# Zhengjun-Du/LC-CRF-SLAM

Hardware: AMD Instinct MI355X
Metric: CRF mean-field iters/sec (higher is better)
Workload: dtype f32; 1 GPU; C2: 2000 keypoints, 5 iters, two 2-D kernels (TUM3.yaml), L=2; frames_in_flight_per_gpu=16384, handles=1, distinct_frames=64, n_points=2000, n_iters=5, n_labels=2, engine=fused

## Files before the change

lc-crf-slam_amd/csrc/fused_lean.h:

```cpp
#pragma once

#include "fused_loop.h"

#ifndef LCCRF_LEAN_SKIP
#define LCCRF_LEAN_SKIP 0
#endif
#define LEAN_SKIP(bit) ((LCCRF_LEAN_SKIP & (bit)) != 0)

namespace lccrf {
namespace fl {

constexpr int kLeanMaxRounds = 4;
__host__ __device__ constexpr int lean_rounds(int nt) { return nt >= 512 ? 3 : 4; }
__host__ __device__ constexpr int lean_max_v(int nt) { return 3 * (nt - 64); }

__host__ __device__ inline int lean_plane_floats(int NA, int V0)
{
    const int top = V0 < kChainTop ? V0 : kChainTop;
    return (NA * kD1 + 11 * top + 3 * (V0 - top) + 16 + 63) & ~63;
}

__host__ __device__ inline bool lean_chain_wanted(int NA, int V0, int row0, int nt)
{
    return row0 >= kChainMinRow && V0 <= chain_max_v(nt) && V0 <= 256 && lean_plane_floats(NA, V0) < 65535;
}

struct LeanTables {
    int val0, val1, nbr, row;
};
__host__ __device__ inline LeanTables lean_tables(size_t &o, int Vk, bool chain)
{
    auto take = [&](size_t bytes) { size_t r = o; o += (bytes + 15) & ~(size_t)15; return (int)r; };
    LeanTables t;
    t.val0 = take((size_t)(Vk + 1) * sizeof(float2));
    t.val1 = take((size_t)(Vk + 1) * sizeof(float2));
    t.nbr = chain ? take((size_t)kD1 * Vk * sizeof(unsigned)) : -1;
    t.row = take((size_t)(Vk + 2) * sizeof(unsigned short));
    return t;
}

__host__ __device__ inline bool layout_lean(int NA, int K, const int *V, int row0, FusedLayout *lay, int nt, size_t lds_limit)
{
    constexpr int D1 = kD1;
    if (NA < 1 || K < 1 || K > kMaxFusedK) return false;
    for (int k = 0; k < K; ++k)
        if (V[k] >= 65535 || V[k] > lean_max_v(nt)) return false;
    if (row0 >= kChainMinRow && !lean_chain_wanted(NA, V[0], row0, nt)) return false;
    const int chain0 = lean_chain_wanted(NA, V[0], row0, nt);
    {
        FusedLayout L{};
        size_t o = 0;
        auto take = [&](size_t bytes) { size_t r = o; o += (bytes + 15) & ~(size_t)15; return (int)r; };
        L.prod_all = 0;
        L.chain0 = chain0;
        L.zero = take(128);
        size_t shared_prod = 0;
        for (int k = 0; k < K; ++k) {
            const bool chain = k == 0 && chain0;
            L.Ecap[k] = chain ? lean_plane_floats(NA, V[k]) : ((NA * D1 + 63) & ~63);
            const LeanTables lt = lean_tables(o, V[k], chain);
            L.val[k][0] = lt.val0;
            L.val[k][1] = lt.val1;
            L.nbr[k] = lt.nbr;
            L.row[k] = lt.row;
            const size_t pb = (size_t)L.Ecap[k] * 2 * sizeof(float);
            shared_prod = pb > shared_prod ? pb : shared_prod;
        }
        if (o > 65535) return false;
        L.pstart = chain0 ? take((size_t)(V[0] + 2) * sizeof(unsigned short)) : 0;
        const int p = take(shared_prod < 1024 ? 1024 : shared_prod);
        for (int k = 0; k < K; ++k) L.prod[k] = p;
        L.total = (int)o;
        if (o <= lds_limit) {
            *lay = L;
            return true;
        }
    }
    return false;
}

#define LCCRF_ASM_SEL(off, vlo, vhi, S)                                                                             \
    "v_cmp_lt_i32_e32 vcc, " #off ", %[rem]\n\tv_cndmask_b32_e32 %[" #S "], 0, %[ad], vcc\n\t"                     \
    "ds_read_b128 v[" #vlo ":" #vhi "], %[" #S "] offset:" #off "\n\t"

__device__ __forceinline__ float chain_rows_sel(unsigned addr, int bytes, unsigned trips, unsigned &keep0, unsigned &keep1)
{
    float acc = 0.0f;
    if (trips == 0) return acc;
    unsigned sa, sb;
    asm volatile(
        LCCRF_ASM_SEL(0, 96, 99, sa) LCCRF_ASM_SEL(16, 100, 103, sb)
        LCCRF_ASM_SEL(32, 104, 107, sa) LCCRF_ASM_SEL(48, 108, 111, sb)
        LCCRF_ASM_SEL(64, 112, 115, sa) LCCRF_ASM_SEL(80, 116, 119, sb)
        "1:\n\t"
        LCCRF_ASM_SEL(96, 120, 123, sa) LCCRF_ASM_SEL(112, 124, 127, sb)
        "s_waitcnt lgkmcnt(6)\n\t"
        LCCRF_ASM_ADD8(v96, v97, v98, v99, v100, v101, v102, v103)
        "v_add_u32_e32 %[ad], 0x80, %[ad]\n\t"
        "v_subrev_u32_e32 %[rem], 0x80, %[rem]\n\t"
        LCCRF_ASM_SEL(0, 96, 99, sa) LCCRF_ASM_SEL(16, 100, 103, sb)
        "s_waitcnt lgkmcnt(6)\n\t"
        LCCRF_ASM_ADD8(v104, v105, v106, v107, v108, v109, v110, v111)
        LCCRF_ASM_SEL(32, 104, 107, sa) LCCRF_ASM_SEL(48, 108, 111, sb)
        "s_waitcnt lgkmcnt(6)\n\t"
        LCCRF_ASM_ADD8(v112, v113, v114, v115, v116, v117, v118, v119)
        LCCRF_ASM_SEL(64, 112, 115, sa) LCCRF_ASM_SEL(80, 116, 119, sb)
        "s_waitcnt lgkmcnt(6)\n\t"
        LCCRF_ASM_ADD8(v120, v121, v122, v123, v124, v125, v126, v127)
        "s_sub_u32 %[n], %[n], 1\n\t"
        "s_cmp_lg_u32 %[n], 0\n\t"
        "s_cbranch_scc1 1b\n\t"
        "s_waitcnt lgkmcnt(0)\n\t"
        : [acc] "+v"(acc), [ad] "+v"(addr), [rem] "+v"(bytes), [n] "+s"(trips), [sa] "=&v"(sa), [sb] "=&v"(sb), "+v"(keep0), "+v"(keep1)
        :
        : "scc", "vcc", "memory", LCCRF_CHAIN_RING_CLOBBERS);
    return acc;
}

__device__ __forceinline__ float chain_rows_keep(unsigned addr, unsigned end, unsigned trips, unsigned &keep0, unsigned &keep1)
{
    float acc = 0.0f;
    if (trips == 0) return acc;
    const unsigned e1 = end - 32u, e2 = end - 64u, e3 = end - 96u;
    unsigned sel;
    asm volatile(LCCRF_CHAIN_ROWS_ASM
                 : [acc] "+v"(acc), [ad] "+v"(addr), [n] "+s"(trips), [sel] "=&v"(sel), "+v"(keep0), "+v"(keep1)
                 : [e0] "v"(end), [e1] "v"(e1), [e2] "v"(e2), [e3] "v"(e3)
                 : "scc", "memory", LCCRF_CHAIN_RING_CLOBBERS);
    return acc;
}

__device__ __forceinline__ float2 lds_f2(unsigned addr)
{
#if defined(__HIP_DEVICE_COMPILE__)
    typedef float lean_f2 __attribute__((ext_vector_type(2)));
    const lean_f2 v = *reinterpret_cast<const __attribute__((address_space(3))) lean_f2 *>((unsigned long)addr);
    return make_float2(v.x, v.y);
#else
    (void)addr;
    return make_float2(0.f, 0.f);
#endif
}

__device__ __forceinline__ void lds_store_f(unsigned addr, float v)
{
#if defined(__HIP_DEVICE_COMPILE__)
    *reinterpret_cast<__attribute__((address_space(3))) float *>((unsigned long)addr) = v;
#else
    (void)addr; (void)v;
#endif
}
__device__ __forceinline__ void lds_store_f2(unsigned addr, float a, float b)
{
#if defined(__HIP_DEVICE_COMPILE__)
    typedef float lean_f2 __attribute__((ext_vector_type(2)));
    lean_f2 v;
    v.x = a;
    v.y = b;
    *reinterpret_cast<__attribute__((address_space(3))) lean_f2 *>((unsigned long)addr) = v;
#else
    (void)addr; (void)a; (void)b;
#endif
}

template <int PPT, int K, int CH>
__device__ __forceinline__ void point_products_lean(const FusedLayout &lay, const PointRegs<PPT, K> &pr, int s, int k)
{
    const unsigned a0 = (pr.ix[s][k][1] >> 16) << 2, a1 = (pr.ix[s][k][2] & 0xffffu) << 2, a2 = (pr.ix[s][k][2] >> 16) << 2;
    if (chain_k<CH>(lay, k)) {
        const unsigned pb = (unsigned)lay.Ecap[k] * 4u;
        lds_store_f(a0, pr.bary[s][k][0] * pr.q[s].x);
        lds_store_f(a0 + pb, pr.bary[s][k][0] * pr.q[s].y);
        lds_store_f(a1, pr.bary[s][k][1] * pr.q[s].x);
        lds_store_f(a1 + pb, pr.bary[s][k][1] * pr.q[s].y);
        lds_store_f(a2, pr.bary[s][k][2] * pr.q[s].x);
        lds_store_f(a2 + pb, pr.bary[s][k][2] * pr.q[s].y);
    } else {
        lds_store_f2(a0, pr.bary[s][k][0] * pr.q[s].x, pr.bary[s][k][0] * pr.q[s].y);
        lds_store_f2(a1, pr.bary[s][k][1] * pr.q[s].x, pr.bary[s][k][1] * pr.q[s].y);
        lds_store_f2(a2, pr.bary[s][k][2] * pr.q[s].x, pr.bary[s][k][2] * pr.q[s].y);
    }
}

template <int PPT, int K>
__device__ __forceinline__ float2 slice_point_lean(const PointRegs<PPT, K> &pr, int s, int k, float alpha)
{
    const float2 x0 = lds_f2(pr.ix[s][k][0] & 0xffffu), x1 = lds_f2(pr.ix[s][k][0] >> 16), x2 = lds_f2(pr.ix[s][k][1] & 0xffffu);
    const float w0 = pr.bary[s][k][0] * alpha, w1 = pr.bary[s][k][1] * alpha, w2 = pr.bary[s][k][2] * alpha;
    float t0 = w0 * x0.x, t1 = w0 * x0.y;
    t0 += w1 * x1.x; t1 += w1 * x1.y;
    t0 += w2 * x2.x; t1 += w2 * x2.y;
    return make_float2(t0, t1);
}

template <int NT>
__device__ __forceinline__ ChainLane chain_setup_lean(unsigned char *smem, const FusedLayout &lay, int V0, int tid)
{
    constexpr int k = 0;
    ChainLane cl{0u, 0u};
    int *hist = reinterpret_cast<int *>(smem + lay.prod[k]);
    if (tid < 128) hist[tid] = 0;
    __syncthreads();
    const unsigned short *row = reinterpret_cast<const unsigned short *>(smem + lay.row[k]);
    unsigned short *srt = reinterpret_cast<unsigned short *>(smem + lay.prod[k]) + 256;
    unsigned short *pstart = reinterpret_cast<unsigned short *>(smem + lay.pstart);
    int key = 0;
    if (tid < V0) {
        const int len = (int)row[tid + 1] - (int)row[tid];
        key = 63 - min((len + 3) >> 4, 63);
        atomicAdd(&hist[key], 1);
    }
    __syncthreads();
    if (tid < 64) {
        const int x = hist[tid];
        int incl = x;
#pragma unroll
        for (int o = 1; o < 64; o <<= 1) {
            const int y = __shfl_up(incl, o, 64);
            if (tid >= o) incl += y;
        }
        hist[64 + tid] = incl - x;
    }
    __syncthreads();
    if (tid < V0) srt[atomicAdd(&hist[64 + key], 1)] = (unsigned short)tid;
    __syncthreads();
    if (tid < 64) {
        int sz[4], sum = 0;
#pragma unroll
        for (int u = 0; u < 4; ++u) {
            const int r = tid * 4 + u;
            sz[u] = 0;
            if (r < V0) {
                const int v = srt[r];
                const int rl = (int)row[v + 1] - (int)row[v];
                sz[u] = ((rl + 3) & ~3) + (r < kChainTop ? 8 : 0);
            }
            sum += sz[u];
        }
        int incl = sum;
#pragma unroll
        for (int o = 1; o < 64; o <<= 1) {
            const int y = __shfl_up(incl, o, 64);
            if (tid >= o) incl += y;
        }
        int base = incl - sum;
#pragma unroll
        for (int u = 0; u < 4; ++u) {
            const int r = tid * 4 + u;
            if (r < V0) pstart[srt[r]] = (unsigned short)base;
            base += sz[u];
        }
    }
    __syncthreads();
    const int l = (tid >> 6) & 1, pr = tid >> 7, ln = tid & 63;
    const int r = pr == 0 ? (chain_top_rank(ln) >= 0 ? chain_top_rank(ln) : V0) : kChainTop + ((pr - 1) << 6) + ln;
    unsigned quads = 0, addr = 0;
    if (r < V0) {
        const int v = srt[r];
        const int rl = (int)row[v + 1] - (int)row[v], len4 = (rl + 3) & ~3;
        addr = (unsigned)(lay.prod[k] + 4 * (l * lay.Ecap[k] + (int)pstart[v]));
        quads = (unsigned)(len4 >> 2);
        cl.b = quads | ((unsigned)(len4 - rl) << 13) | ((unsigned)((v + 1) * 2 + l) << 16);
    }
    unsigned m = quads;
#pragma unroll
    for (int o = 32; o > 0; o >>= 1) m = max(m, (unsigned)__shfl_xor((int)m, o));
    cl.a = addr | (m << 18);
    __syncthreads();
    return cl;
}

__device__ __forceinline__ void chain_pads_lean(unsigned char *smem, const ChainLane &cl, int tid)
{
    if (cl.b >> 16) {
        float *e = reinterpret_cast<float *>(smem + (cl.a & 0x3ffffu)) + (cl.b & 0x1fffu) * 4u;
        const unsigned npad = (cl.b >> 13) & 3u;
        for (unsigned z = 1; z <= npad; ++z) e[-(int)z] = 0.0f;
        if ((tid >> 7) == 0) {
            reinterpret_cast<float4 *>(e)[0] = make_float4(0.f, 0.f, 0.f, 0.f);
            reinterpret_cast<float4 *>(e)[1] = make_float4(0.f, 0.f, 0.f, 0.f);
        }
    }
}

template <int PPT, int K, int CH, int NT>
__device__ __forceinline__ void place_products_lean(unsigned char *smem, const FusedLayout &lay, int N, int tid,
                                                    const unsigned (&pk)[PPT][K][kD1], PointRegs<PPT, K> &pr)
{
#pragma unroll
    for (int k = 0; k < K; ++k) {
        const unsigned short *row = reinterpret_cast<const unsigned short *>(smem + lay.row[k]);
        const unsigned short *pstart = reinterpret_cast<const unsigned short *>(smem + lay.pstart);
#pragma unroll
        for (int s = 0; s < PPT; ++s) {
            const unsigned vb = (unsigned)lay.val[k][kD1 & 1];
            pr.ix[s][k][0] = (vb + 8u * (pk[s][k][0] & 0xffffu)) | ((vb + 8u * (pk[s][k][1] & 0xffffu)) << 16);
            pr.ix[s][k][1] = vb + 8u * (pk[s][k][2] & 0xffffu);
            pr.ix[s][k][2] = 0;
            if (tid + s * NT < N) {
                unsigned sl[kD1];
#pragma unroll
                for (int j = 0; j < kD1; ++j) {
                    sl[j] = pk[s][k][j] >> 16;
                    if (chain_k<CH>(lay, k)) {
                        const int v = (int)(pk[s][k][j] & 0xffffu) - 1;
                        sl[j] = (unsigned)((int)pstart[v] + ((int)(pk[s][k][j] >> 16) - (int)row[v]));
                        sl[j] = ((unsigned)lay.prod[k] >> 2) + sl[j];
                    } else {
                        sl[j] = ((unsigned)lay.prod[k] >> 2) + 2u * sl[j];
                    }
                }
                pr.ix[s][k][1] |= sl[0] << 16;
                pr.ix[s][k][2] = sl[1] | (sl[2] << 16);
            }
        }
    }
}

__host__ __device__ inline int lean_sorted_vertex(int q, int V, int nt)
{
    const int r = q / nt;
    int w = (q % nt) >> 6;
    if ((r & 1) && (r + 1) * nt <= V) w = (nt >> 6) - 1 - w;
    return r * nt + (w << 6) + (q & 63);
}

template <int NT>
__device__ __forceinline__ int block_excl_scan(int x, int tid, int *ws)
{
    int incl = x;
#pragma unroll
    for (int o = 1; o < 64; o <<= 1) {
        const int y = __shfl_up(incl, o, 64);
        if ((tid & 63) >= o) incl += y;
    }
    if ((tid & 63) == 63) ws[tid >> 6] = incl;
    __syncthreads();
    int before = 0;
#pragma unroll
    for (int w = 0; w < NT / 64; ++w) {
        const int s = ws[w];
        if (w < (tid >> 6)) before += s;
    }
    return before + incl - x;
}

template <int PPT, int K, int NT>
__device__ __forceinline__ void sort_short_rows(unsigned char *smem, const FusedLayout &lay, int k, int Vk, int tid,
                                                unsigned (&pk)[PPT][K][kD1], const unsigned *gnbr, int Epad, unsigned *out, int axis_words)
{
    constexpr int VM = (lean_max_v(NT) + 8 + 7) & ~7;
    static_assert(NT == 512, "one lane per (bucket, segment): 64 x 8");
    static_assert(4 * VM * 2 + 64 <= ((NT * kD1 + 63) & ~63) * 8, "the scratch fits the smallest product buffer of the plan");
    unsigned short *row = reinterpret_cast<unsigned short *>(smem + lay.row[k]);
    unsigned short *key = reinterpret_cast<unsigned short *>(smem + lay.prod[k]);
    unsigned short *perm = key + VM, *nlen = perm + VM, *nrow = nlen + VM;
    int *ws = reinterpret_cast<int *>(nrow + VM);
    __syncthreads();
    for (int v = tid; v < Vk; v += NT) key[v] = (unsigned short)(63 - min((int)row[v + 1] - (int)row[v], 63));
    __syncthreads();
    const int b = tid >> 3, seg_len = (Vk + 7) >> 3, lo = min((tid & 7) * seg_len, Vk), hi = min(lo + seg_len, Vk);
    int cnt = 0;
    for (int v = lo; v < hi; ++v) cnt += key[v] == b ? 1 : 0;
    int q = block_excl_scan<NT>(cnt, tid, ws);
    for (int v = lo; v < hi; ++v) {
        if (key[v] == b) {
            const int nv = lean_sorted_vertex(q++, Vk, NT);
            perm[v] = (unsigned short)nv;
            nlen[nv] = (unsigned short)((int)row[v + 1] - (int)row[v]);
        }
    }
    __syncthreads();
    {
        int l[3], sum = 0;
#pragma unroll
        for (int i = 0; i < 3; ++i) {
            l[i] = tid * 3 + i < Vk ? (int)nlen[tid * 3 + i] : 0;
            sum += l[i];
        }
        int at = block_excl_scan<NT>(sum, tid, ws + NT / 64);
#pragma unroll
        for (int i = 0; i < 3; ++i) {
            if (tid * 3 + i <= Vk) nrow[tid * 3 + i] = (unsigned short)at;
            at += l[i];
        }
    }
    __syncthreads();
#pragma unroll
    for (int s = 0; s < PPT; ++s) {
#pragma unroll
        for (int j = 0; j < kD1; ++j) {
            const unsigned w = pk[s][k][j], id = w & 0xffffu;
            if (id) {
                const int v = (int)id - 1, nv = perm[v];
                pk[s][k][j] = (unsigned)(nv + 1) | ((unsigned)((int)nrow[nv] + ((int)(w >> 16) - (int)row[v])) << 16);
            }
        }
    }
    for (int j = 0; j < kD1; ++j) {
        for (int v = tid; v < Vk; v += NT) {
            const unsigned n = gnbr[(size_t)j * Epad + v], n1 = n & 0xffffu, n2 = n >> 16;
            out[j * axis_words + perm[v]] = (n1 ? (unsigned)perm[n1 - 1] + 1u : 0u) | ((n2 ? (unsigned)perm[n2 - 1] + 1u : 0u) << 16);
        }
    }
    __syncthreads();
    for (int v = tid; v <= Vk; v += NT) row[v] = nrow[v];
    __syncthreads();
}

typedef unsigned lean_u3 __attribute__((ext_vector_type(3)));
struct LeanSrc {
    __amdgpu_buffer_rsrc_t nbr[kMaxFusedK];
    __amdgpu_buffer_rsrc_t bary[kMaxFusedK];
    __amdgpu_buffer_rsrc_t norm[kMaxFusedK];
    __amdgpu_buffer_rsrc_t unary;
    int nbr_axis_bytes[kMaxFusedK];
    int off_nbr[kMaxFusedK], off_bary[kMaxFusedK], off_norm[kMaxFusedK], off_unary;
};
constexpr int kLeanRecPoints = 4 * kNTSmall;
constexpr int kLeanRecUnary = 0;
constexpr int kLeanRecBary = kLeanRecUnary + kLeanRecPoints * 8;
constexpr int kLeanRecNorm = kLeanRecBary + kMaxFusedK * kLeanRecPoints * kD1 * 4;
constexpr int kLeanRecNbr = kLeanRecNorm + kMaxFusedK * kLeanRecPoints * 4;
constexpr int kLeanRecNbrAxis = lean_max_v(kNTSmall) * 4;
constexpr int kLeanRecBytes = (kLeanRecNbr + kD1 * kLeanRecNbrAxis + 255) & ~255;
__device__ __forceinline__ __amdgpu_buffer_rsrc_t lean_rsrc(const void *p, size_t bytes)
{
    return __builtin_amdgcn_make_buffer_rsrc(const_cast<void *>(p), 0, (int)bytes, 0x00020000);
}

template <int PPT, int K>
__device__ __forceinline__ void opaque_ids(PointRegs<PPT, K> &pr)
{
#pragma unroll
    for (int s = 0; s < PPT; ++s) {
#pragma unroll
        for (int k = 0; k < K; ++k) asm volatile("" : "+v"(pr.ix[s][k][0]), "+v"(pr.ix[s][k][1]), "+v"(pr.ix[s][k][2]));
    }
}

struct LeanPrepPlan {
    int cl_off;
    int row_off[kMaxFusedK], row_bytes[kMaxFusedK];
    int nbr_off[kMaxFusedK], nbr_bytes[kMaxFusedK];
    int snbr_off[kMaxFusedK], snbr_axis[kMaxFusedK];
    int total;
};
constexpr unsigned kLeanPrepFormat = 7;
__host__ __device__ inline LeanPrepPlan lean_prep_plan(const FusedLayout &lay, int K, const int *Vcap, int nt, int ppt, bool sorted = false)
{
    LeanPrepPlan p{};
    int o = K * ppt * nt * 12;
    p.cl_off = o;
    o += nt * 8;
    for (int k = 0; k < K; ++k) {
        p.row_off[k] = o;
        p.row_bytes[k] = ((Vcap[k] + 2) * 2 + 15) & ~15;
        o += p.row_bytes[k];
        p.nbr_off[k] = o;
        p.nbr_bytes[k] = lay.nbr[k] >= 0 ? ((kD1 * Vcap[k] * 4 + 15) & ~15) : 0;
        o += p.nbr_bytes[k];
    }
    for (int k = 0; k < K; ++k) {
        p.snbr_off[k] = o;
        p.snbr_axis[k] = (sorted && lay.nbr[k] < 0) ? ((Vcap[k] + 3) & ~3) * 4 : 0;
        o += kD1 * p.snbr_axis[k];
    }
    p.total = (o + 255) & ~255;
    return p;
}

template <int PPT, int K, int CH, int NT, bool RELOAD, bool NORM = false, bool PRELOADED = false>
__device__ __forceinline__ void mean_field_lean(unsigned char *smem, const FusedLayout &lay, const int (&V)[K], int N, int &t,
                                                PointRegs<PPT, K> &pr, ChainLane &cl, const float (&alpha)[K],
                                                const float (&wk)[K], const LeanSrc &src, int n_iter, float relax, float omr, Instr &ins)
{
    constexpr int D1 = kD1;
    constexpr int KF = K - 1;
    const int wave_base = __builtin_amdgcn_readfirstlane(t & ~63);
    (void)wave_base;
#define LEAN_FRESH_T()                                                                                               \
    do {                                                                                                             \
        int z_ = 0;                                                                                                  \
        asm volatile("" : "+v"(z_));                                                                                 \
        t = wave_base + (int)__builtin_amdgcn_mbcnt_hi(~0u, __builtin_amdgcn_mbcnt_lo(~0u, (unsigned)z_));          \
    } while (0)
    auto load_weights = [&]() {
        if (!RELOAD) return;
#pragma unroll
        for (int s = 0; s < PPT; ++s) {
            const int i = t + s * NT;
            if (!NORM) {
                typedef unsigned lean_u2 __attribute__((ext_vector_type(2)));
                const lean_u2 u = __builtin_amdgcn_raw_buffer_load_b64(src.unary, i * 8, src.off_unary, 0);
                pr.un[s] = make_float2(__uint_as_float(u.x), __uint_as_float(u.y));
            }
#pragma unroll
            for (int k = 0; k < K; ++k) {
                const lean_u3 b = __builtin_amdgcn_raw_buffer_load_b96(src.bary[k], i * (D1 * 4), src.off_bary[k], 0);
                pr.bary[s][k][0] = __uint_as_float(b.x);
                pr.bary[s][k][1] = __uint_as_float(b.y);
                pr.bary[s][k][2] = __uint_as_float(b.z);
                if (!NORM) pr.wn[s][k] = __uint_as_float(__builtin_amdgcn_raw_buffer_load_b32(src.norm[k], i * 4, src.off_norm[k], 0));
            }
        }
        if (NORM) return;
#pragma unroll
        for (int s = 0; s < PPT; ++s)
#pragma unroll
            for (int k = 0; k < K; ++k) pr.wn[s][k] = wk[k] * pr.wn[s][k];
    };
    auto phase_P = [&](int k) {
#pragma unroll
        for (int s = 0; s < PPT; ++s)
            if (t + s * NT < N) point_products_lean<PPT, K, CH>(lay, pr, s, k);
        if (chain_k<CH>(lay, k)) chain_pads_lean(smem, cl, t);
    };
    auto phase_S = [&](int k) {
        float *val = reinterpret_cast<float *>(smem + lay.val[k][0]);
        if (chain_k<CH>(lay, k)) {
            const int npairs = 1 + ((max(V[k] - kChainTop, 0) + 63) >> 6);
            if (__builtin_expect((t >> 7) < npairs, 1)) {
                FL_PSTAMP();
                if ((t >> 7) == 0) __builtin_amdgcn_s_setprio(3);
                asm volatile("" : "+v"(cl.a), "+v"(cl.b));
                if (__builtin_expect((cl.b >> 16) != 0, 1) && !LEAN_SKIP(2)) {
                    const unsigned row_addr = cl.a & 0x3ffffu, row_end = row_addr + (cl.b & 0x1fffu) * 16u;
                    const unsigned m = (unsigned)__builtin_amdgcn_readfirstlane((int)(cl.a >> 18));
                    const float acc = (t >> 7) == 0 ? chain_rows_keep(row_addr, row_end, (((m + 1u) >> 1) + 3u) >> 2, cl.a, cl.b)
                                                      : chain_rows_sel(row_addr, (int)((cl.b & 0x1fffu) * 16u), (m + 7u) >> 3, cl.a, cl.b);
                    val[cl.b >> 16] = acc;
                }
                LEAN_FRESH_T();
                if ((t >> 7) == 0) __builtin_amdgcn_s_setprio(0);
                FL_PSTAMP();
            }
            return;
        }
        if (LEAN_SKIP(32)) return;
        const float2 *pl = reinterpret_cast<const float2 *>(smem + lay.prod[k]);
        const float2 *zero = reinterpret_cast<const float2 *>(smem + lay.zero);
        const unsigned short *row = reinterpret_cast<const unsigned short *>(smem + lay.row[k]);
        constexpr int RS = (K == 2 && CH == 0) ? 1 : lean_rounds(NT);
        for (int base = 0; base < lean_rounds(NT); base += RS) {
            int p0[RS], pe[RS];
#pragma unroll
            for (int r = 0; r < RS; ++r) {
                const int v = t + (base + r) * NT;
                p0[r] = pe[r] = 0;
                if (v < V[k]) { p0[r] = row[v]; pe[r] = row[v + 1]; }
            }
            float2 x[RS][8];
#pragma unroll
            for (int r = 0; r < RS; ++r) {
                const unsigned base = (unsigned)lay.prod[k] + 8u * (unsigned)p0[r];
                const int n = pe[r] - p0[r];
#pragma unroll
                for (int u = 0; u < 8; ++u) x[r][u] = lds_f2(((u < n) ? base : 0u) + 8u * u);
            }
#pragma unroll
            for (int r = 0; r < RS; ++r) {
                const int v = t + (base + r) * NT;
                float a0 = 0.0f, a1 = 0.0f;
#pragma unroll
                for (int u = 0; u < 8; ++u) { a0 += x[r][u].x; a1 += x[r][u].y; }
                for (int p = p0[r] + 8; p < pe[r] && !LEAN_SKIP(16); p += 8) {
                    float2 y[8];
#pragma unroll
                    for (int u = 0; u < 8; ++u) y[u] = *((p + u < pe[r]) ? pl + p + u : zero);
#pragma unroll
                    for (int u = 0; u < 8; ++u) { a0 += y[u].x; a1 += y[u].y; }
                }
                if (v < V[k]) reinterpret_cast<float2 *>(val)[v + 1] = make_float2(a0, a1);
            }
        }
        (void)V;
    };
    constexpr int R = lean_rounds(NT);
    constexpr int OVL_K = (K == 2 && CH == 1) ? 1 : K;
    auto load_nbr = [&](unsigned (&w)[OVL_K][D1][R]) {
#pragma unroll
        for (int k = 0; k < K; ++k) {
#pragma unroll
            for (int j = 0; j < D1; ++j) {
#pragma unroll
                for (int r = 0; r < R; ++r) {
                    w[k][j][r] = 0;
                    if (!(CH == 1 && k == 0) && (r == 0 || r * NT < V[k]))
                        w[k][j][r] = __builtin_amdgcn_raw_buffer_load_b32(src.nbr[k], (t + r * NT) * 4, src.off_nbr[k] + j * src.nbr_axis_bytes[k], 0);
                }
            }
        }
    };
    auto blur_pass = [&](int j, const unsigned (&w)[OVL_K][D1][R]) {
#pragma unroll
        for (int k = 0; k < K; ++k) {
            const float2 *src_v = reinterpret_cast<const float2 *>(smem + lay.val[k][j & 1]);
            float2 *dst = reinterpret_cast<float2 *>(smem + lay.val[k][(j & 1) ^ 1]);
            const bool in_lds = CH == 1 && k == 0;
            const unsigned *lds = reinterpret_cast<const unsigned *>(smem + (in_lds ? lay.nbr[k] : 0)) + j * V[k];
#pragma unroll
            for (int r = 0; r < (in_lds ? 1 : R); ++r) {
                const int v = t + r * NT;
                if (v < V[k]) {
                    const unsigned n = in_lds ? lds[v] : w[k][j][r];
                    const float2 o = src_v[v + 1], x = src_v[n & 0xffffu], y = src_v[n >> 16];
                    float2 u;
                    u.x = o.x + 0.5f * (x.x + y.x);
                    u.y = o.y + 0.5f * (x.y + y.y);
                    dst[v + 1] = u;
                }
            }
        }
    };
    constexpr bool OVL = K == 2 && CH == 1;
    constexpr int NA0 = NT - 128, RA = 4;
    constexpr int NB = NT - 64, RB = 3;
    auto load_nbr_ovl = [&](unsigned (&wa)[RA], unsigned (&wb)[2][RB]) {
#pragma unroll
        for (int r = 0; r < RA; ++r) {
            wa[r] = 0;
            if ((r == 0 || r * NA0 < V[K - 1]) && !LEAN_SKIP(512))
                wa[r] = __builtin_amdgcn_raw_buffer_load_b32(src.nbr[K - 1], (t - 128 + r * NA0) * 4, src.off_nbr[K - 1], 0);
        }
#pragma unroll
        for (int j = 1; j < D1; ++j) {
#pragma unroll
            for (int r = 0; r < RB; ++r) {
                wb[j - 1][r] = 0;
                if ((r == 0 || r * NB < V[K - 1]) && !LEAN_SKIP(512))
                    wb[j - 1][r] = __builtin_amdgcn_raw_buffer_load_b32(src.nbr[K - 1], (t + r * NB) * 4, src.off_nbr[K - 1] + j * src.nbr_axis_bytes[K - 1], 0);
            }
        }
    };
    auto blur_vertex = [&](const float2 *src_v, float2 *dst, int v, unsigned n) {
        if (LEAN_SKIP(64)) return;
        const float2 o = src_v[v + 1], x = src_v[n & 0xffffu], y = src_v[n >> 16];
        float2 u;
        u.x = o.x + 0.5f * (x.x + y.x);
        u.y = o.y + 0.5f * (x.y + y.y);
        dst[v + 1] = u;
    };
    auto blur_big = [&](int j, int lane, int stride, int rounds, const unsigned *w) {
        constexpr int k = K - 1;
        const float2 *src_v = reinterpret_cast<const float2 *>(smem + lay.val[k][j & 1]);
        float2 *dst = reinterpret_cast<float2 *>(smem + lay.val[k][(j & 1) ^ 1]);
#pragma unroll
        for (int r = 0; r < RA; ++r) {
            if (r < rounds) {
                const int v = lane + r * stride;
                if (v < V[k]) blur_vertex(src_v, dst, v, w[r]);
            }
        }
    };
    auto blur_small = [&](int lane, int j_lo, int j_hi) {
        const unsigned *tbl = reinterpret_cast<const unsigned *>(smem + lay.nbr[0]);
#pragma unroll
        for (int j = 0; j < D1; ++j) {
            if (j < j_lo || j >= j_hi) continue;
            const float2 *src_v = reinterpret_cast<const float2 *>(smem + lay.val[0][j & 1]);
            float2 *dst = reinterpret_cast<float2 *>(smem + lay.val[0][(j & 1) ^ 1]);
            for (int v = lane; v < V[0]; v += 64) blur_vertex(src_v, dst, v, tbl[j * V[0] + v]);
            asm volatile("s_waitcnt lgkmcnt(0)" ::: "memory");
            __builtin_amdgcn_wave_barrier();
        }
    };
    auto point_update = [&](int s) {
        if constexpr (NORM) {
#pragma unroll
            for (int k = 0; k < K; ++k) {
                const float v = slice_point_lean(pr, s, k, alpha[k]).x;
                const float nrm = 1.0f / (v + 1e-20f);
                if (RELOAD) __builtin_amdgcn_raw_buffer_store_b32(__float_as_uint(nrm), src.norm[k], (t + s * NT) * 4, src.off_norm[k], 0);
                else pr.wn[s][k] = wk[k] * nrm;
            }
            return;
        }
        float nx[2] = {-pr.un[s].x, -pr.un[s].y};
#pragma unroll
        for (int k = 0; k < K; ++k) {
            const float2 t = slice_point_lean(pr, s, k, alpha[k]);
            nx[0] += pr.wn[s][k] * t.x;
            nx[1] += pr.wn[s][k] * t.y;
        }
        pr.q[s] = softmax2(nx[0], nx[1], pr.q[s], relax, omr);
    };

    if (n_iter <= 0) return;
    if (!PRELOADED) load_weights();
#pragma unroll
    for (int s = 0; s < PPT; ++s)
        if (t + s * NT < N) point_products_lean<PPT, K, CH>(lay, pr, s, KF);
    if (chain_k<CH>(lay, KF)) chain_pads_lean(smem, cl, t);
    for (int it = 0; it < n_iter; ++it) {
        LEAN_FRESH_T();
        if (RELOAD) opaque_ids(pr);
        else opaque(pr);
        unsigned w[OVL ? 1 : K][D1][R];
        unsigned wa[RA], wb[2][RB];
        if constexpr (OVL) load_nbr_ovl(wa, wb);
        else load_nbr(w);
        __syncthreads();
        FL_STAMP();
        phase_S(KF);
#pragma unroll
        for (int k = KF - 1; k >= 0; --k) {
            __syncthreads();
            opaque_ids(pr);
            phase_P(k);
            __syncthreads();
            phase_S(k);
        }
        if constexpr (OVL) {
            if (t >= 128) blur_big(0, t - 128, NA0, RA, wa);
            __syncthreads();
            FL_STAMP();
            LEAN_FRESH_T();
            if (t >= NB) blur_small(t - NB, 0, 2);
            else blur_big(1, t, NB, RB, wb[0]);
            __syncthreads();
            if (!NORM && !LEAN_SKIP(256)) load_weights();
            if (t < NB) blur_big(2, t, NB, RB, wb[1]);
            else blur_small(t - NB, 2, D1);
            __syncthreads();
        } else {
            __syncthreads();
            FL_STAMP();
            LEAN_FRESH_T();
            blur_pass(0, w);
            __syncthreads();
            blur_pass(1, w);
            __syncthreads();
            if (!NORM && !LEAN_SKIP(256)) load_weights();
            blur_pass(2, w);
            __syncthreads();
        }
        FL_STAMP();
        LEAN_FRESH_T();
        opaque_ids(pr);
        const bool more = it + 1 < n_iter;
#pragma unroll
        for (int s = 0; s < PPT; ++s) {
            if (t + s * NT < N && !LEAN_SKIP(128)) {
                point_update(s);
                if (more) point_products_lean<PPT, K, CH>(lay, pr, s, KF);
            }
        }
        FL_STAMP();
    }
}

#undef LEAN_FRESH_T

}
}
```

Baseline: 49.93 million iters/s.

## Split chain rows across one wave with half-wave lanes, freeing a wave for blur

Remaps the chain-sum (phase_S) work so that each 64-lane wave handles 32 chain rows, two lanes per row for the two labels, instead of a wave pair covering 64 rows. The chain therefore uses one wave for the top rows rather than two. The first blur pass on the other lattice can then start at thread 64 instead of 128 and needs three rounds instead of four. This is meant to put more threads on the overlapped blur and shorten the critical path. In exchange each chain lane handles fewer distinct rows, and the prep format version is bumped because the lane layout changed.

Result: faster. 50.57 million iters/s, median of 6 (+1.3%).

```diff
diff --git a/lc-crf-slam_amd/csrc/fused_lean.h b/lc-crf-slam_amd/csrc/fused_lean.h
--- a/lc-crf-slam_amd/csrc/fused_lean.h
+++ b/lc-crf-slam_amd/csrc/fused_lean.h
@@ -10,13 +10,18 @@
 namespace lccrf {
 namespace fl {
 
+#ifndef LCCRF_CHAIN_TOP
+#define LCCRF_CHAIN_TOP 16
+#endif
+constexpr int kLeanChainTop = LCCRF_CHAIN_TOP;
+static_assert(kLeanChainTop == kChainTop || kLeanChainTop == 32, "16 rows on the lanes chain_top_rank names, or a full wavefront");
 constexpr int kLeanMaxRounds = 4;
 __host__ __device__ constexpr int lean_rounds(int nt) { return nt >= 512 ? 3 : 4; }
 __host__ __device__ constexpr int lean_max_v(int nt) { return 3 * (nt - 64); }
 
 __host__ __device__ inline int lean_plane_floats(int NA, int V0)
 {
-    const int top = V0 < kChainTop ? V0 : kChainTop;
+    const int top = V0 < kLeanChainTop ? V0 : kLeanChainTop;
     return (NA * kD1 + 11 * top + 3 * (V0 - top) + 16 + 63) & ~63;
 }
 
@@ -193,6 +198,18 @@
     return make_float2(t0, t1);
 }
 
+__host__ __device__ constexpr int lean_chain_row(int tid)
+{
+    const int w = tid >> 6, ln = tid & 63;
+    if (w == 0 && kLeanChainTop < 32) {
+        const int r = chain_top_rank(ln & ~16);
+        return r >= 0 ? (r | (((ln >> 4) & 1) << 16)) : -1;
+    }
+    return (w == 0 ? (ln & 31) : kLeanChainTop + ((w - 1) << 5) + (ln & 31)) | ((ln >> 5) << 16);
+}
+__host__ __device__ constexpr int lean_chain_waves(int V0) { return 1 + (((V0 > kLeanChainTop ? V0 - kLeanChainTop : 0) + 31) >> 5); }
+static_assert(lean_chain_waves(chain_max_v(kNTSmall)) <= kNTSmall / 64, "every chain row of the plan has a lane");
+
 template <int NT>
 __device__ __forceinline__ ChainLane chain_setup_lean(unsigned char *smem, const FusedLayout &lay, int V0, int tid)
 {
@@ -233,7 +250,7 @@
             if (r < V0) {
                 const int v = srt[r];
                 const int rl = (int)row[v + 1] - (int)row[v];
-                sz[u] = ((rl + 3) & ~3) + (r < kChainTop ? 8 : 0);
+                sz[u] = ((rl + 3) & ~3) + (r < kLeanChainTop ? 8 : 0);
             }
             sum += sz[u];
         }
@@ -252,8 +269,8 @@
         }
     }
     __syncthreads();
-    const int l = (tid >> 6) & 1, pr = tid >> 7, ln = tid & 63;
-    const int r = pr == 0 ? (chain_top_rank(ln) >= 0 ? chain_top_rank(ln) : V0) : kChainTop + ((pr - 1) << 6) + ln;
+    const int cr = lean_chain_row(tid);
+    const int l = cr >> 16, r = cr < 0 ? V0 : (cr & 0xffff);
     unsigned quads = 0, addr = 0;
     if (r < V0) {
         const int v = srt[r];
@@ -276,7 +293,7 @@
         float *e = reinterpret_cast<float *>(smem + (cl.a & 0x3ffffu)) + (cl.b & 0x1fffu) * 4u;
         const unsigned npad = (cl.b >> 13) & 3u;
         for (unsigned z = 1; z <= npad; ++z) e[-(int)z] = 0.0f;
-        if ((tid >> 7) == 0) {
+        if ((tid >> 6) == 0) {
             reinterpret_cast<float4 *>(e)[0] = make_float4(0.f, 0.f, 0.f, 0.f);
             reinterpret_cast<float4 *>(e)[1] = make_float4(0.f, 0.f, 0.f, 0.f);
         }
@@ -446,7 +463,7 @@
     int snbr_off[kMaxFusedK], snbr_axis[kMaxFusedK];
     int total;
 };
-constexpr unsigned kLeanPrepFormat = 7;
+constexpr unsigned kLeanPrepFormat = 8;
 __host__ __device__ inline LeanPrepPlan lean_prep_plan(const FusedLayout &lay, int K, const int *Vcap, int nt, int ppt, bool sorted = false)
 {
     LeanPrepPlan p{};
@@ -519,20 +536,20 @@
     auto phase_S = [&](int k) {
         float *val = reinterpret_cast<float *>(smem + lay.val[k][0]);
         if (chain_k<CH>(lay, k)) {
-            const int npairs = 1 + ((max(V[k] - kChainTop, 0) + 63) >> 6);
-            if (__builtin_expect((t >> 7) < npairs, 1)) {
+            const int nwaves = lean_chain_waves(V[k]);
+            if (__builtin_expect((t >> 6) < nwaves, 1)) {
                 FL_PSTAMP();
-                if ((t >> 7) == 0) __builtin_amdgcn_s_setprio(3);
+                if ((t >> 6) == 0) __builtin_amdgcn_s_setprio(3);
                 asm volatile("" : "+v"(cl.a), "+v"(cl.b));
                 if (__builtin_expect((cl.b >> 16) != 0, 1) && !LEAN_SKIP(2)) {
                     const unsigned row_addr = cl.a & 0x3ffffu, row_end = row_addr + (cl.b & 0x1fffu) * 16u;
                     const unsigned m = (unsigned)__builtin_amdgcn_readfirstlane((int)(cl.a >> 18));
-                    const float acc = (t >> 7) == 0 ? chain_rows_keep(row_addr, row_end, (((m + 1u) >> 1) + 3u) >> 2, cl.a, cl.b)
+                    const float acc = (t >> 6) == 0 ? chain_rows_keep(row_addr, row_end, (((m + 1u) >> 1) + 3u) >> 2, cl.a, cl.b)
                                                       : chain_rows_sel(row_addr, (int)((cl.b & 0x1fffu) * 16u), (m + 7u) >> 3, cl.a, cl.b);
                     val[cl.b >> 16] = acc;
                 }
                 LEAN_FRESH_T();
-                if ((t >> 7) == 0) __builtin_amdgcn_s_setprio(0);
+                if ((t >> 6) == 0) __builtin_amdgcn_s_setprio(0);
                 FL_PSTAMP();
             }
             return;
@@ -614,14 +631,16 @@
         }
     };
     constexpr bool OVL = K == 2 && CH == 1;
-    constexpr int NA0 = NT - 128, RA = 4;
+    constexpr int A0 = 64;
+    constexpr int NA0 = NT - A0, RA = 3;
+    static_assert(RA * NA0 >= lean_max_v(NT), "three rounds cover the plan's largest lattice");
     constexpr int NB = NT - 64, RB = 3;
     auto load_nbr_ovl = [&](unsigned (&wa)[RA], unsigned (&wb)[2][RB]) {
 #pragma unroll
         for (int r = 0; r < RA; ++r) {
             wa[r] = 0;
             if ((r == 0 || r * NA0 < V[K - 1]) && !LEAN_SKIP(512))
-                wa[r] = __builtin_amdgcn_raw_buffer_load_b32(src.nbr[K - 1], (t - 128 + r * NA0) * 4, src.off_nbr[K - 1], 0);
+                wa[r] = __builtin_amdgcn_raw_buffer_load_b32(src.nbr[K - 1], (t - A0 + r * NA0) * 4, src.off_nbr[K - 1], 0);
         }
 #pragma unroll
         for (int j = 1; j < D1; ++j) {
@@ -712,7 +731,7 @@
             phase_S(k);
         }
         if constexpr (OVL) {
-            if (t >= 128) blur_big(0, t - 128, NA0, RA, wa);
+            if (t >= A0) blur_big(0, t - A0, NA0, RA, wa);
             __syncthreads();
             FL_STAMP();
             LEAN_FRESH_T();
```
